# rdesc/autorally

Measured on AMD Instinct MI355X. Metric: trajectory rollouts/s per MPPI solve, higher is better.
Workload: dtype f32

## Files before the change

autorally_amd/capi.py:

```python
import ctypes as C
import os

import numpy as np

HERE = os.path.dirname(os.path.abspath(__file__))
LIB_PATH = os.environ.get("MPPI_LIB_PATH") or os.path.join(HERE, "libmppi_hip.so")
MAX_LAYERS = 8

OK, ERR_INVALID, ERR_NO_DEVICE, ERR_HIP, ERR_STATE, ERR_UNSUPPORTED = range(6)


class Config(C.Structure):
    _fields_ = [
        ("device", C.c_int),
        ("num_rollouts", C.c_int),
        ("num_timesteps", C.c_int),
        ("hz", C.c_int),
        ("optimization_stride", C.c_int),
        ("gamma", C.c_float),
        ("num_iters", C.c_int),
        ("n_layers", C.c_int),
        ("layers", C.c_int * MAX_LAYERS),
        ("exploration_std", C.c_float * 2),
        ("init_control", C.c_float * 2),
# ... 5 lines not shown


class CostParams(C.Structure):
    _fields_ = [(n, C.c_float) for n in (
        "desired_speed", "speed_coeff", "track_coeff", "max_slip_ang", "slip_penalty", "track_slop",
        "crash_coeff", "steering_coeff", "throttle_coeff", "boundary_threshold", "discount")] + [
        ("l1_cost", C.c_int)]


class StageTimes(C.Structure):
    _fields_ = [("n_solves", C.c_int), ("noise_ms", C.c_float), ("rollout_ms", C.c_float),
                ("weights_ms", C.c_float), ("reduction_ms", C.c_float), ("total_ms", C.c_float)]


SYMBOLS = [
    "mppi_abi_version", "mppi_strerror", "mppi_last_error", "mppi_device_count", "mppi_create",
    "mppi_destroy", "mppi_set_nn_params", "mppi_update_model", "mppi_set_control_limits",
    "mppi_set_costmap", "mppi_set_costmap_transform", "mppi_set_costmap_channel", "mppi_set_cost_params", "mppi_reset_controls",
    "mppi_set_control_seq", "mppi_get_control_seq", "mppi_set_control_hist", "mppi_get_control_hist",
    "mppi_savitsky_golay", "mppi_slide_control_seq", "mppi_seed", "mppi_set_noise", "mppi_generate_noise",
    "mppi_compute_control", "mppi_control_ticks", "mppi_compute_control_async", "mppi_synchronize",
    "mppi_compute_control_batch_async", "mppi_compute_control_batch", "mppi_control_ticks_batch", "mppi_get_results",
    "mppi_get_applied_controls", "mppi_rollout_only", "mppi_nominal_traj", "mppi_nominal_traj_pair",
    "mppi_set_bf_params", "mppi_set_ddp_weights", "mppi_debug_cost_raster", "mppi_compute_feedback_gains", "mppi_get_feedback_gains",
    "mppi_enable_stage_timing", "mppi_reset_stage_times", "mppi_get_stage_times",
    "mppi_rollout_variant", "mppi_set_rollout_variant", "mppi_debug_dynamics",
    "mppi_debug_inject_handover_fault", "mppi_compute_feedback_gains_pair", "mppi_set_host_threads",
    "mppi_debug_capture_iterations", "mppi_debug_get_iterations", "mppi_set_wait_timeout", "mppi_debug_form_candidates",
    "mppi_debug_set_chained_ticks", "mppi_debug_min_cost",
    "mppi_arm", "mppi_arm_batch", "mppi_disarm", "mppi_is_armed", "mppi_debug_launch_info",
    "mppi_trace_rollouts", "mppi_top_rollouts",
    "mppi_compute_feedback_gains_batch", "mppi_debug_ddp_info", "mppi_debug_device_tanhf",
    "mppi_nominal_traj_batch", "mppi_debug_nominal_info",
]

ABI2_SYMBOLS = ("mppi_debug_inject_handover_fault", "mppi_savitsky_golay", "mppi_set_costmap_transform",
                "mppi_compute_control_batch", "mppi_compute_control_batch_async", "mppi_control_ticks_batch",
                "mppi_nominal_traj_pair")
ABI3_SYMBOLS = ("mppi_compute_feedback_gains_pair", "mppi_set_host_threads")
ABI4_SYMBOLS = ("mppi_debug_capture_iterations", "mppi_debug_get_iterations", "mppi_set_wait_timeout", "mppi_debug_form_candidates")
ABI5_SYMBOLS = ("mppi_debug_set_chained_ticks", "mppi_debug_min_cost", "mppi_arm", "mppi_arm_batch", "mppi_disarm",
                "mppi_is_armed")

UNVERSIONED_SYMBOLS = ("mppi_debug_launch_info", "mppi_trace_rollouts", "mppi_top_rollouts",
                       "mppi_compute_feedback_gains_batch", "mppi_debug_ddp_info", "mppi_debug_device_tanhf",
                       "mppi_nominal_traj_batch", "mppi_debug_nominal_info")

_lib = None


class MppiError(RuntimeError):
    def __init__(self, status, msg):
        super().__init__("mppi status %d: %s" % (status, msg))
        self.status = status


def lib():
    global _lib
    if _lib is None:
        if not os.path.exists(LIB_PATH):
            raise RuntimeError("libmppi_hip.so is missing: run `python -m autorally_amd.build` "
                               "or __graft_entry__.build() first")
        L = C.CDLL(LIB_PATH)
        fp = C.POINTER(C.c_float)
        hp = C.c_void_p
        L.mppi_abi_version.restype = C.c_int
        L.mppi_strerror.restype = C.c_char_p
        L.mppi_strerror.argtypes = [C.c_int]
        L.mppi_last_error.restype = C.c_char_p
        L.mppi_last_error.argtypes = [hp]
        L.mppi_device_count.restype = C.c_int
        L.mppi_create.argtypes = [C.POINTER(Config), C.POINTER(hp)]
        L.mppi_destroy.argtypes = [hp]
        L.mppi_set_nn_params.argtypes = [hp, fp, C.c_size_t]
        L.mppi_update_model.argtypes = [hp, C.POINTER(C.c_int), C.c_int, fp, C.c_size_t]
        L.mppi_set_control_limits.argtypes = [hp, fp, fp]
        L.mppi_set_costmap.argtypes = [hp, C.c_int, C.c_int, fp, fp, fp, fp]
        L.mppi_set_costmap_transform.argtypes = [hp, fp, fp, fp]
        L.mppi_set_costmap_channel.argtypes = [hp, C.c_int, fp, C.c_size_t]
# ... 38 lines not shown
        v3 = L.mppi_abi_version() >= 3
        if v3:
            L.mppi_compute_feedback_gains_pair.argtypes = [hp, fp, fp, fp, hp, fp, fp, fp]
            L.mppi_set_host_threads.argtypes = [C.c_int]
        v4 = L.mppi_abi_version() >= 4
        if v4:
            L.mppi_debug_capture_iterations.argtypes = [hp, C.c_int]
            L.mppi_debug_get_iterations.argtypes = [hp, fp, fp, fp]
            L.mppi_set_wait_timeout.argtypes = [hp, C.c_double]
            L.mppi_debug_form_candidates.argtypes = [hp, C.POINTER(C.c_char_p), C.c_int]
        v5 = L.mppi_abi_version() >= 5
        if v5:
            L.mppi_debug_set_chained_ticks.argtypes = [hp, C.c_int]
            L.mppi_debug_min_cost.argtypes = [hp, C.c_int, C.POINTER(C.c_int)]
            L.mppi_arm.argtypes = [hp, C.c_double]
            L.mppi_arm_batch.argtypes = [C.POINTER(hp), C.c_int, C.c_double]
            L.mppi_disarm.argtypes = [hp]
            L.mppi_is_armed.argtypes = [hp]
        if hasattr(L, "mppi_debug_launch_info"):
            L.mppi_debug_launch_info.argtypes = [hp, C.POINTER(C.c_int), C.POINTER(C.c_int)]
        if hasattr(L, "mppi_trace_rollouts"):
            ip = C.POINTER(C.c_int)
            L.mppi_trace_rollouts.argtypes = [hp, ip, C.c_int, fp, fp, fp, fp, ip]
            L.mppi_top_rollouts.argtypes = [hp, C.c_int, ip]
        if hasattr(L, "mppi_compute_feedback_gains_batch"):
            fpp = C.POINTER(fp)
            L.mppi_compute_feedback_gains_batch.argtypes = [C.POINTER(hp), fp, fpp, fpp, C.c_int]
            L.mppi_debug_ddp_info.argtypes = [hp, C.POINTER(C.c_int)]
            L.mppi_debug_device_tanhf.argtypes = [C.c_int, fp, fp, C.c_size_t]
        if hasattr(L, "mppi_nominal_traj_batch"):
            fpp = C.POINTER(fp)
            L.mppi_nominal_traj_batch.argtypes = [C.POINTER(hp), fp, fpp, fpp, C.c_int]
            L.mppi_debug_nominal_info.argtypes = [hp, C.POINTER(C.c_int)]
        for s in SYMBOLS:
            if (v2 or s not in ABI2_SYMBOLS) and (v3 or s not in ABI3_SYMBOLS) and (v4 or s not in ABI4_SYMBOLS) and \
                    (v5 or s not in ABI5_SYMBOLS) and s not in UNVERSIONED_SYMBOLS:
                getattr(L, s)
        _lib = L
    return _lib


def _fp(a):
    return a.ctypes.data_as(C.POINTER(C.c_float))


def _f32(a, shape=None):
    a = np.ascontiguousarray(a, dtype=np.float32)
    if shape is not None:
        a = a.reshape(shape)
    return a


def make_config_struct(cfg, device=0):
    c = Config()
    c.device = int(device)
    c.num_rollouts = int(cfg["K"])
    c.num_timesteps = int(cfg["T"])
    c.hz = int(cfg["hz"])
    c.optimization_stride = int(cfg["opt_stride"])
    c.gamma = float(cfg["gamma"])
    c.num_iters = int(cfg.get("num_iters", 1))
    layers = [] if cfg.get("bf_W") is not None else [int(x) for x in cfg["layers"]]
    c.n_layers = len(layers)
    for i, v in enumerate(layers):
        c.layers[i] = v
    for i in range(2):
# ... 140 lines not shown
        self._ck(self.L.mppi_debug_min_cost(self.h, int(on), C.byref(got)))
        return bool(got.value)

    def arm(self, max_wait_s=0.01):
        self._ck(self.L.mppi_arm(self.h, float(max_wait_s)))

    def disarm(self):
        self._ck(self.L.mppi_disarm(self.h))

    def is_armed(self):
        return bool(self.L.mppi_is_armed(self.h))

    def debug_launch_info(self):
        n, g = C.c_int(-1), C.c_int(-1)
        self._ck(self.L.mppi_debug_launch_info(self.h, C.byref(n), C.byref(g)))
        return n.value, g.value

    def compute_control_async(self, state):
        self._ck(self.L.mppi_compute_control_async(self.h, _fp(_f32(state, (7,)))))

    def synchronize(self):
        self._ck(self.L.mppi_synchronize(self.h))

    def get_results(self, with_vectors=True):
        U = np.zeros((self.T, 2), dtype=np.float32)
        tc = C.c_float()
        costs = np.zeros(self.K, dtype=np.float32) if with_vectors else None
        w = np.zeros(self.K, dtype=np.float32) if with_vectors else None
        self._ck(self.L.mppi_get_results(self.h, _fp(U), C.byref(tc),
                                         _fp(costs) if with_vectors else None,
                                         _fp(w) if with_vectors else None))
        return dict(U=U, traj_cost=tc.value, costs=costs, w=w)

    def get_applied_controls(self):
        V = np.zeros((self.K, self.T, 2), dtype=np.float32)
        self._ck(self.L.mppi_get_applied_controls(self.h, _fp(V), V.size))
        return V

    def trace_rollouts(self, ks, with_costs=True):
        ks = np.ascontiguousarray(ks, dtype=np.int32).reshape(-1)
        n = ks.size
        out = dict(states=np.zeros((n, self.T, 7), np.float32), controls=np.zeros((n, self.T, 2), np.float32),
                   first_crash=np.zeros(n, np.int32))
        if with_costs:
            out.update(step_costs=np.zeros((n, self.T), np.float32), costs=np.zeros(n, np.float32))
        ip = C.POINTER(C.c_int)
        self._ck(self.L.mppi_trace_rollouts(self.h, ks.ctypes.data_as(ip), n, _fp(out["states"]), _fp(out["controls"]),
                                            _fp(out["step_costs"]) if with_costs else None,
                                            _fp(out["costs"]) if with_costs else None, out["first_crash"].ctypes.data_as(ip)))
        return out

    def top_rollouts(self, n):
        ks = np.zeros(int(n), np.int32)
        self._ck(self.L.mppi_top_rollouts(self.h, int(n), ks.ctypes.data_as(C.POINTER(C.c_int))))
        return ks

    def rollout_only(self, state):
        costs = np.zeros(self.K, dtype=np.float32)
        self._ck(self.L.mppi_rollout_only(self.h, _fp(_f32(state, (7,))), _fp(costs)))
        return costs

    def nominal_traj(self, state):
        ss = np.zeros((self.T, 7), dtype=np.float32)
        cs = np.zeros((self.T, 2), dtype=np.float32)
        self._ck(self.L.mppi_nominal_traj(self.h, _fp(_f32(state, (7,))), _fp(ss), _fp(cs)))
        return ss, cs
# ... 186 lines not shown
```

autorally_amd/csrc/abi_host.hip:

```cpp
#include "abi_internal.hpp"

#include <stdexcept>

using namespace mppi;
using namespace mppi_abi;

namespace mppi_abi {

class HostHelper {
 public:
  ~HostHelper()
  {
    if (!th_.joinable()) return;
    {
      std::lock_guard<std::mutex> lk(mu_);
      quit_ = true;
      wake_ = true;
    }
    cv_.notify_one();
    th_.join();
  }
  void arm()
  {
    std::call_once(started_, [this] { th_ = std::thread([this] { loop(); }); });
// ... 530 lines not shown
  for (int at = 0; at < n; at += kMaxFleet) {
    const int m = std::min(kMaxFleet, n - at);
    const int rcm = ddp_fleet_launch(handles + at, states + (size_t)MPPI_STATE_DIM * at, xs.data() + at, us.data() + at, m);
    if (rcm == MPPI_ERR_HIP) return rcm;
    if (rcm && !rc) rc = rcm;
  }
  return rc;
}

int mppi_debug_ddp_info(const mppi_handle *h, int *on_device)
{
  if (!h || !on_device) return MPPI_ERR_INVALID;
  *on_device = h->ddp_on_device;
  return MPPI_OK;
}

int mppi_debug_device_tanhf(int device, const float *in, float *out, size_t n)
{
  if (device < 0 || !in || !out || n == 0) return MPPI_ERR_INVALID;
  hipDeviceProp_t prop;
  if (hipGetDeviceProperties(&prop, device) != hipSuccess || strncmp(prop.gcnArchName, "gfx950", 6) != 0) return MPPI_ERR_NO_DEVICE;
  if (ensure_device(device) != hipSuccess) return MPPI_ERR_HIP;
  float *d_in = nullptr, *d_out = nullptr;
  hipError_t e = hipMalloc(reinterpret_cast<void **>(&d_in), sizeof(float) * n);
  if (e == hipSuccess) e = hipMalloc(reinterpret_cast<void **>(&d_out), sizeof(float) * n);
  if (e == hipSuccess) e = hipMemcpy(d_in, in, sizeof(float) * n, hipMemcpyHostToDevice);
  if (e == hipSuccess) e = launch_device_tanhf(d_in, d_out, n, nullptr);
  if (e == hipSuccess) e = hipMemcpy(out, d_out, sizeof(float) * n, hipMemcpyDeviceToHost);
  if (d_in) (void)hipFree(d_in);
  if (d_out) (void)hipFree(d_out);
  return e == hipSuccess ? MPPI_OK : MPPI_ERR_HIP;
}

int mppi_set_host_threads(int n)
{
  if (n < 1 || n > 2) return MPPI_ERR_INVALID;
  g_host_threads.store(n, std::memory_order_relaxed);
  if (n >= 2) host_helper().arm();
  return MPPI_OK;
}

int mppi_get_feedback_gains(mppi_handle *h, float *feedback, float *feedforward, float *state_traj,
                            float *control_traj, float *total_cost)
{
  if (!h) return MPPI_ERR_INVALID;
  if (!h->have_ddp) return fail(h, MPPI_ERR_STATE, "mppi_compute_feedback_gains has not succeeded yet");
  const DdpResult &r = h->ddp;
  if (feedback) memcpy(feedback, r.feedback.data(), sizeof(float) * r.feedback.size());
  if (feedforward) memcpy(feedforward, r.feedforward.data(), sizeof(float) * r.feedforward.size());
  if (state_traj) memcpy(state_traj, r.x.data(), sizeof(float) * r.x.size());
  if (control_traj) memcpy(control_traj, r.u.data(), sizeof(float) * r.u.size());
  if (total_cost) *total_cost = r.total_cost;
  return MPPI_OK;
}

}
```

autorally_amd/csrc/abi_solve.hip:

```cpp
#include "abi_internal.hpp"

using namespace mppi;
using namespace mppi_abi;

namespace mppi_abi {

std::mutex g_batch_mu;
hipStream_t g_batch_stream[64] = {};
hipStream_t batch_stream(int device)
{
  if (device < 0 || device >= 64) return nullptr;
  std::lock_guard<std::mutex> lk(g_batch_mu);
  if (!g_batch_stream[device] &&
      hipStreamCreateWithFlags(&g_batch_stream[device], hipStreamNonBlocking) != hipSuccess)
    g_batch_stream[device] = nullptr;
  return g_batch_stream[device];
}

hipError_t arg_block_create(ArgBlock &b, size_t slot_bytes)
{
  b.slot = (slot_bytes + 255) & ~(size_t)255;
  hipError_t e = hipMalloc(reinterpret_cast<void **>(&b.d), b.slot);
  if (e == hipSuccess) e = hipHostMalloc(reinterpret_cast<void **>(&b.h), b.slot * ArgBlock::kRing, hipHostMallocDefault);
  for (int i = 0; i < ArgBlock::kRing && e == hipSuccess; i++) e = hipEventCreateWithFlags(&b.ev[i], hipEventDisableTiming);
// ... 1150 lines not shown
}

int mppi_rollout_only(mppi_handle *h, const float state[MPPI_STATE_DIM], float *costs)
{
  int rc = check_ready(h);
  if (rc) return rc;
  if (!state || !costs) return fail(h, MPPI_ERR_INVALID, "NULL argument");
  DISARM(h);
  HIPCHK(h, hipSetDevice(h->cfg.device));
  rc = recover_timed_out(h);
  if (rc) return rc;
  rc = mppi_synchronize(h);
  if (rc) return rc;
  OWN(h);
  rc = upload_controls_if_dirty(h, h->stream);
  if (rc) return rc;
  float *noise = nullptr;
  bool in_kernel = false;
  rc = eps_source(h, Eps::Single, 0, &noise, &in_kernel, nullptr);
  if (rc) return rc;
  h->explicit_iters = 0;
  forget_solve_state(h);
  RolloutArgs a;
  fill_rollout_args(h, state, noise, a);
  if (in_kernel) use_inline_noise(h, a);
  rc = launch_rollout(h, a);
  if (rc) return rc;
  note_solve_state(h, state, false);
  HIPCHK(h, hipMemcpyAsync(costs, h->d_costs, sizeof(float) * h->K, hipMemcpyDeviceToHost, h->stream));
  HIPCHK(h, hipStreamSynchronize(h->stream));
  return MPPI_OK;
}

int mppi_debug_capture_iterations(mppi_handle *h, int on)
{
  if (!h) return MPPI_ERR_INVALID;
  DISARM(h);
  int rc = mppi_synchronize(h);
  if (rc) return rc;
  if (on && !h->d_cap) {
    HIPCHK(h, hipSetDevice(h->cfg.device));
    HIPCHK(h, hipMalloc(&h->d_cap, sizeof(float) * (size_t)h->cfg.num_iters * (2 * (size_t)h->T + h->K)));
  }
  h->capture = on != 0;
  h->cap_valid = false;
  return MPPI_OK;
}

int mppi_debug_get_iterations(mppi_handle *h, float *U_raw, float *costs, float *V)
{
  if (!h) return MPPI_ERR_INVALID;
  int rc = mppi_synchronize(h);
  if (rc) return rc;
  if (!h->cap_valid) return fail(h, MPPI_ERR_STATE, "no captured solve (mppi_debug_capture_iterations, then a solve on this handle alone)");
  if (V && !h->cap_explicit) return fail(h, MPPI_ERR_STATE, "applied controls of every iteration exist for explicit-noise solves only");
  const int iters = h->cfg.num_iters, T = h->T, K = h->K;
  HIPCHK(h, hipSetDevice(h->cfg.device));
  OWN(h);
  HIPCHK(h, hipStreamSynchronize(h->stream));
  const size_t rec = 2 * (size_t)T + K;
  std::vector<float> buf((size_t)iters * rec);
  HIPCHK(h, hipMemcpy(buf.data(), h->d_cap, sizeof(float) * buf.size(), hipMemcpyDeviceToHost));
  for (int it = 0; it < iters; it++) {
    if (U_raw) {
      float *u = U_raw + (size_t)it * 2 * T;
      if (it < iters - 1) memcpy(u, buf.data() + (size_t)it * rec, sizeof(float) * 2 * (size_t)T);
// ... 77 lines not shown
```

autorally_amd/csrc/mppi_device.hpp:

```cpp
#pragma once

#include <hip/hip_runtime.h>
#include <stdint.h>

namespace mppi {

constexpr int kStateDim = 7;
constexpr int kControlDim = 2;
constexpr int kNetIn = 6;
constexpr int kNetOut = 4;
constexpr int kRolloutsPerWave = 16;

struct CostArgs {
  float desired_speed, speed_coeff, track_coeff, max_slip_ang, slip_penalty, track_slop;
  float crash_coeff, steering_coeff, throttle_coeff, boundary_threshold;
  float crash_cost_discounted;
  int l1_cost;
  float r_c1[3], r_c2[3], trs[3];
  int affine;
  int need_control_cost;
  int map_w, map_h;
  const float *map;
};

// ... 126 lines not shown
  return r;
}

__device__ __forceinline__ float tanh_fast(float x)
{
  const float e = __builtin_amdgcn_exp2f(x * 2.88539008177792681472f);
  const float r = __builtin_amdgcn_rcpf(e + 1.0f);
  return fmaf(-2.0f, r, 1.0f);
}

constexpr float kTanhScale = 2.88539008177792681472f;
__device__ __forceinline__ float tanh_bias(float z, float bs)
{
  const float e = __builtin_amdgcn_exp2f(fmaf(z, kTanhScale, bs));
  const float r = __builtin_amdgcn_rcpf(e + 1.0f);
  return fmaf(-2.0f, r, 1.0f);
}

typedef float f32x2 __attribute__((ext_vector_type(2)));
typedef float f32x4 __attribute__((ext_vector_type(4)));
__device__ __forceinline__ f32x2 tanh_bias2(f32x2 z, f32x2 bs)
{
  const f32x2 y = __builtin_elementwise_fma(z, f32x2{kTanhScale, kTanhScale}, bs);
  f32x2 e;
  e.x = __builtin_amdgcn_exp2f(y.x);
  e.y = __builtin_amdgcn_exp2f(y.y);
  const f32x2 d = e + f32x2{1.0f, 1.0f};
  f32x2 r;
  r.x = __builtin_amdgcn_rcpf(d.x);
  r.y = __builtin_amdgcn_rcpf(d.y);
  return __builtin_elementwise_fma(f32x2{-2.0f, -2.0f}, r, f32x2{1.0f, 1.0f});
}

__device__ __forceinline__ void sincos_fast(float x, float &sn, float &cs)
{
  const double xd = (double)x;
  const double q = rint(xd * 0.63661977236758134308);
  double rd = fma(-q, 1.5707963267948966, xd);
  rd = fma(-q, 6.123233995736766e-17, rd);
  const float r = (float)rd;
  const float r2 = r * r;
  const float ps = fmaf(fmaf(-1.9515295891e-4f, r2, 8.3321608736e-3f), r2, -1.6666654611e-1f);
  const float s0 = fmaf(r * r2, ps, r);
  const float pc = fmaf(fmaf(2.443315711809948e-5f, r2, -1.388731625493765e-3f), r2, 4.166664568298827e-2f);
  const float c0 = fmaf(r2 * r2, pc, fmaf(r2, -0.5f, 1.0f));
  const int qi = (int)q;
  const float a = (qi & 1) ? c0 : s0;
  const float b = (qi & 1) ? s0 : c0;
  sn = (qi & 2) ? -a : a;
  cs = ((qi + 1) & 2) ? -b : b;
}

template <bool AFFINE>
__device__ __forceinline__ unsigned texel_index(const CostArgs &c, float x, float y)
{
  float u = fmaf(c.r_c1[0], x, c.r_c2[0] * y) + c.trs[0];
  float v = fmaf(c.r_c1[1], x, c.r_c2[1] * y) + c.trs[1];
  if (!AFFINE) {
    const float w = fmaf(c.r_c1[2], x, c.r_c2[2] * y) + c.trs[2];
    u = u / w;
    v = v / w;
  }
  float fi = floorf(u * (float)c.map_w);
  float fj = floorf(v * (float)c.map_h);
  fi = fminf(fmaxf(fi, 0.0f), (float)(c.map_w - 1));
  fj = fminf(fmaxf(fj, 0.0f), (float)(c.map_h - 1));
// ... 136 lines not shown
```

autorally_amd/csrc/mppi_kernels.hpp:

```cpp
#pragma once
#include "mppi_device.hpp"

#include <hip/hip_ext.h>
#include <atomic>
#include <type_traits>

namespace mppi {

extern thread_local hipEvent_t tl_kernel_start, tl_kernel_stop;
#define MPPI_LAUNCH_ROLLOUT(kern, grid, block, lds, stream, ...)                                                   \
  do {                                                                                                             \
    if (::mppi::tl_kernel_start != nullptr)                                                                        \
      hipExtLaunchKernelGGL(kern, grid, block, lds, stream, ::mppi::tl_kernel_start, ::mppi::tl_kernel_stop, 0,    \
                            __VA_ARGS__);                                                                          \
    else                                                                                                           \
      hipLaunchKernelGGL(kern, grid, block, lds, stream, __VA_ARGS__);                                             \
  } while (0)

template <class F>
inline hipError_t dispatch_cost_flags(bool affine, bool ctrl, F &&f)
{
  if (affine && !ctrl) return f(std::true_type{}, std::false_type{});
  if (affine && ctrl) return f(std::true_type{}, std::true_type{});
  if (!affine && !ctrl) return f(std::false_type{}, std::false_type{});
// ... 197 lines not shown
  int *first_crash;
  int n, K, T;
  float nu[2], u_lo[2], u_hi[2], dt;
  int negate_yaw_der;
  CostArgs cost;
};
bool trace_image_in_lds(const NetDesc &net);
hipError_t launch_rollout_trace(const NetDesc &net, const TraceArgs &a, hipStream_t stream);
hipError_t launch_rollout_trace_bf(const TraceArgs &a, hipStream_t stream);

struct TailLaunch {
  const float *costs, *V, *hist;
  float *U, *w, *scal, *res, *slid;
  unsigned *counter;
  int K, T, last_iter, slide_stride;
  unsigned seq;
  float gamma, init0, init1;
  unsigned long long *ug = nullptr;
  int no_device_copy = 0;
  float *hist_out = nullptr;
  unsigned long long *gx = nullptr, *gpart = nullptr;
  unsigned epoch = 0, poll_ticks = 0;
  int fault = 0;
  const unsigned long long *min_cost = nullptr;
  unsigned min_cost_tag = 0;
};
bool tail_is_stream(int K);
constexpr int kTailExchangeGranules = 3 * 64 + 32 * 16 + 32 * 64;
hipError_t launch_solve_tail(const TailLaunch &l, hipStream_t stream);
hipError_t launch_solve_tail_batch(const TailLaunch *l, int n, hipStream_t stream);
size_t solve_tail_fleet_arg_bytes();
void fill_solve_tail_fleet(void *dst, const TailLaunch *l, int n);
hipError_t launch_solve_tail_fleet(const TailLaunch *l, int n, const void *d_args, hipStream_t stream);
hipError_t launch_debug_cost(const CostArgs &c, float x, float y, float heading, int width_m, int height_m,
                             int ppm, float *out, hipStream_t stream);
hipError_t launch_slide(float *in, int T, int stride, float init0, float init1, hipStream_t stream);
hipError_t launch_kt_to_tk(const float *src, float *dst, int K, int T, hipStream_t stream);
hipError_t launch_tk_to_kt(const float *src, float *dst, int K, int T, hipStream_t stream);

hipError_t launch_noise(const uint32_t *rng_in, uint32_t *rng_out, const uint32_t *jump, int K, int T,
                        int L, int C, float *eps, hipStream_t stream);
struct NoiseFleetDesc {
  const uint32_t *rng_in;
  uint32_t *rng_out;
  const uint32_t *jump;
  float *eps;
  int K, T, L, C;
};
hipError_t launch_noise_fleet(const NoiseFleetDesc *h_desc, const NoiseFleetDesc *d_desc, int n, hipStream_t stream);
hipError_t launch_noise_init(uint32_t *rng, int K, const uint32_t base[6], const uint32_t *sub,
                             int sub_bits, const uint32_t *one, uint64_t offset, hipStream_t stream);

struct DdpFleetArgs {
  const float *theta;
  const float *wimg;
  const float *in;
  float *out, *work;
  int T, negate_yaw_der;
  int img_lds;
  float dt;
  float u_lo[2], u_hi[2], Q[7], R[2], Qf[7];
  NetDesc net;
};
__host__ __device__ inline int ddp_fleet_hidden(const NetDesc &net)
{
  int s = 0;
// ... 27 lines not shown
```

autorally_amd/csrc/solve_kernels.hip:

```cpp
#include "mppi_device.hpp"
#include "mppi_kernels.hpp"


namespace mppi {


#ifdef MPPI_TAIL_STAMPS
__device__ unsigned long long g_tail_stamps[16];
#define TSTAMP(i)                                                                                   \
  do {                                                                                              \
    if (block == T / 2 && threadIdx.x == 0) {                                                       \
      unsigned long long t__;                                                                       \
      asm volatile("s_memrealtime %0\n\ts_waitcnt lgkmcnt(0)" : "=s"(t__)::"memory");               \
      g_tail_stamps[i] = t__;                                                                       \
    }                                                                                               \
  } while (0)
#else
#define TSTAMP(i) do { } while (0)
#endif
#ifndef MPPI_TAIL_THREADS
#define MPPI_TAIL_THREADS 512
#endif
constexpr int kTailThreads = MPPI_TAIL_THREADS;
constexpr int kRedChunk = 4096;

__device__ __forceinline__ float wave_min(float v) { return wave_reduce<true>(v); }
__device__ __forceinline__ float wave_sum(float v) { return wave_reduce<false>(v); }
template <bool MIN>
__device__ __forceinline__ float block_reduce(float v, float *red4)
{
  const int lane = threadIdx.x & 63, wv = threadIdx.x >> 6;
  v = wave_reduce<MIN>(v);
  if (lane == 0) red4[wv] = v;
  __syncthreads();
  float r = red4[0];
#pragma unroll
  for (int i = 1; i < kTailThreads / 64; i++) r = MIN ? fminf(r, red4[i]) : r + red4[i];
  return r;
}

__device__ __forceinline__ void publish_entry(float *res, int entry, float v0, float v1, unsigned seq)
{
  const f32x4 v = {v0, __uint_as_float(seq), v1, __uint_as_float(seq)};
  float *p = res + 4 * (size_t)entry;
  asm volatile("global_store_dwordx4 %0, %1, off sc0 sc1" ::"v"(p), "v"(v) : "memory");
}

__device__ __forceinline__ unsigned long long make_granule(unsigned epoch, float v)
{
  return ((unsigned long long)epoch << 32) | (unsigned long long)__float_as_uint(v);
}
__device__ __forceinline__ void store_granule(unsigned long long *g, unsigned epoch, float v)
{
  __hip_atomic_store(g, make_granule(epoch, v), __ATOMIC_RELAXED, __HIP_MEMORY_SCOPE_AGENT);
}

struct TailArgs {
  const float *costs;
  const float *V;
  float *U;
  const float *hist;
  float *w;
  float *scal;
  float *res;
  int no_device_copy;
  float *hist_out;
  unsigned long long *ug;
  unsigned *counter;
  int K, T;
  float gamma;
  float *slid;
// ... 79 lines not shown
      a.slid[2 * T + tid] = hv;
    }
  }
}

__device__ __forceinline__ void solve_tail_body(const TailArgs &a, const int block, const float *V, const float *costs_p, const int K,
                                                const int T)
{
  constexpr int kGS = 68, kPlane = (kRedChunk / 64) * kGS;
  __shared__ __attribute__((aligned(16))) float tile[2][kPlane];
  __shared__ __attribute__((aligned(16))) float wtile[kPlane];
  __shared__ float redm[kTailThreads / 64], reds[kTailThreads / 64], redt[kTailThreads / 64];
  __shared__ int is_last;
  extern __shared__ __attribute__((aligned(16))) float dyn[];
  float *partial = dyn;
  const int tid = threadIdx.x;
  const bool extra = (block == T);
  const int t = extra ? 0 : block;
  constexpr int base = 0;
  const int n = K;
  TSTAMP(0);

  const float *row = V + ((size_t)t * K + base) * 2;
  constexpr int kPre = kRedChunk / 2 / kTailThreads;
  float4 pre[kPre];
  {
    const float4 *src0 = reinterpret_cast<const float4 *>(row);
#pragma unroll
    for (int i = 0; i < kPre; i++) {
      const int q = tid + i * kTailThreads;
      pre[i] = (q < n / 2) ? src0[q] : make_float4(0, 0, 0, 0);
    }
  }
  float eta;
  {
    constexpr int kCostV = kRedChunk / 4 / kTailThreads;
    const float4 *c4 = reinterpret_cast<const float4 *>(costs_p);
    const int K4 = K / 4;
    float4 cv[kCostV];
#pragma unroll
    for (int i = 0; i < kCostV; i++) {
      const int q = i * kTailThreads + tid;
      cv[i] = (q < K4) ? c4[q] : make_float4(INFINITY, INFINITY, INFINITY, INFINITY);
    }
    float m = INFINITY;
    TSTAMP(1);
#pragma unroll
    for (int i = 0; i < kCostV; i++) m = fminf(fminf(m, fminf(cv[i].x, cv[i].y)), fminf(cv[i].z, cv[i].w));
    TSTAMP(2);
    const float beta = block_reduce<true>(m, redm);
    TSTAMP(3);
    float part = 0.0f;
#pragma unroll
    for (int i = 0; i < kCostV; i++) {
      const int q = i * kTailThreads + tid;
      if (q < K4) {
        const float e0 = expf(-a.gamma * (cv[i].x - beta));
        const float e1 = expf(-a.gamma * (cv[i].y - beta));
        const float e2 = expf(-a.gamma * (cv[i].z - beta));
        const float e3 = expf(-a.gamma * (cv[i].w - beta));
        cv[i] = make_float4(e0, e1, e2, e3);
        part += (e0 + e1) + (e2 + e3);
      }
    }
    TSTAMP(4);
    eta = block_reduce<false>(part, reds);
    TSTAMP(5);
    if (extra) {
      float tc = 0.0f;
#pragma unroll
      for (int i = 0; i < kCostV; i++) {
        const int q = i * kTailThreads + tid;
        if (q < K4) {
          reinterpret_cast<float4 *>(a.w)[q] = cv[i];
          tc += cv[i].x * cv[i].x / eta;
          tc += cv[i].y * cv[i].y / eta;
          tc += cv[i].z * cv[i].z / eta;
          tc += cv[i].w * cv[i].w / eta;
        }
      }
      const float traj = block_reduce<false>(tc, redt);
      if (tid == 0) {
        __hip_atomic_store(&a.scal[0], beta, __ATOMIC_RELAXED, __HIP_MEMORY_SCOPE_AGENT);
        __hip_atomic_store(&a.scal[1], eta, __ATOMIC_RELAXED, __HIP_MEMORY_SCOPE_AGENT);
        __hip_atomic_store(&a.scal[2], traj, __ATOMIC_RELAXED, __HIP_MEMORY_SCOPE_AGENT);
        if (a.last_iter) {
          publish_entry(a.res, T, beta, eta, a.seq);
          publish_entry(a.res, T + 1, traj, 0.0f, a.seq);
        }
      }
    } else {
#pragma unroll
      for (int i = 0; i < kCostV; i++) {
        const int q = i * kTailThreads + tid;
        const int kl = 4 * q - base;
        if (q < K4 && kl >= 0 && kl < n)
          *reinterpret_cast<float4 *>(&wtile[(kl >> 6) * kGS + (kl & 63)]) =
              make_float4(cv[i].x / eta, cv[i].y / eta, cv[i].z / eta, cv[i].w / eta);
      }
    }
  }

  const int G = K / 64;
  if (!extra) {
#pragma unroll
    for (int i = 0; i < kPre; i++) {
      const int q = tid + i * kTailThreads;
      if (q < n / 2) {
        const int kk = 2 * q;
        const int o = (kk >> 6) * kGS + (kk & 63);
        *reinterpret_cast<float2 *>(&tile[0][o]) = make_float2(pre[i].x, pre[i].z);
        *reinterpret_cast<float2 *>(&tile[1][o]) = make_float2(pre[i].y, pre[i].w);
      }
    }
    TSTAMP(6);
    __syncthreads();
    TSTAMP(7);
    for (int c = tid; c < (n / 64) * 2; c += kTailThreads) {
      const int ml = c >> 1, j = c & 1;
      const float4 *p4 = reinterpret_cast<const float4 *>(&tile[j][ml * kGS]);
      const float4 *w4 = reinterpret_cast<const float4 *>(&wtile[ml * kGS]);
      float acc = 0.0f;
#pragma unroll
      for (int i = 0; i < 16; i++) {
        const float4 wv = w4[i], pv = p4[i];
        acc = fmaf(wv.x, pv.x, acc);
        acc = fmaf(wv.y, pv.y, acc);
        acc = fmaf(wv.z, pv.z, acc);
        acc = fmaf(wv.w, pv.w, acc);
      }
      partial[j * G + ml] = acc;
    }
    TSTAMP(8);
    __syncthreads();
  }
  float u = 0.0f;
  if (tid < 2 && !extra) {
    const float *pj = partial + tid * G;
    int mm = 0;
    if ((G & 3) == 0) {
      for (; mm + 32 <= G; mm += 32) {
        float4 v[8];
#pragma unroll
        for (int i = 0; i < 8; i++) v[i] = *reinterpret_cast<const float4 *>(pj + mm + 4 * i);
#pragma unroll
        for (int i = 0; i < 8; i++) { u += v[i].x; u += v[i].y; u += v[i].z; u += v[i].w; }
      }
    }
    for (; mm < G; mm++) u += pj[mm];
    if (a.last_iter) store_granule(a.ug + t * 2 + tid, a.seq, u);
    else a.U[t * 2 + tid] = u;
  }
  if (tid < 64) {
    const float u1 = __shfl(u, 1);
    TSTAMP(9);
    if (tid == 0 && !extra && a.last_iter) publish_entry(a.res, t, u, u1, a.seq);
    TSTAMP(10);
  }
  tail_arrive_and_smooth(a, K, T, (unsigned)(T + 1), is_last, dyn);
}

#ifdef MPPI_TAIL_STAMPS
// ... 337 lines not shown
  }
  SSTAMP(9);
  __syncthreads();
  float u = 0.0f;
  if (tid < 2) {
    const float *pj = partial + tid * G;
    int mm = 0;
    if ((G & 3) == 0 && G >= 32) {
      float4 v[8], w[8];
#pragma unroll
      for (int i = 0; i < 8; i++) v[i] = *reinterpret_cast<const float4 *>(pj + 4 * i);
      for (; mm + 32 <= G; mm += 32) {
        const int nx = (mm + 64 <= G) ? mm + 32 : mm;
#pragma unroll
        for (int i = 0; i < 8; i++) w[i] = *reinterpret_cast<const float4 *>(pj + nx + 4 * i);
#pragma unroll
        for (int i = 0; i < 8; i++) { u += v[i].x; u += v[i].y; u += v[i].z; u += v[i].w; }
#pragma unroll
        for (int i = 0; i < 8; i++) v[i] = w[i];
      }
    }
    for (; mm < G; mm++) u += pj[mm];
    if (a.last_iter) store_granule(a.ug + t * 2 + tid, a.seq, u);
    else a.U[t * 2 + tid] = u;
  }
  if (tid < 64) {
    const float u1 = __shfl(u, 1);
    if (tid == 0 && a.last_iter) publish_entry(a.res, t, u, u1, a.seq);
    SSTAMP(10);
  }
  tail_arrive_and_smooth(a, K, T, (unsigned)T, is_last, img);
}

__global__ __launch_bounds__(kTailThreads) void solve_tail_kernel(const float *V, const float *costs, const int K, const int T,
                                                                  const TailArgs a)
{
  solve_tail_body(a, (int)blockIdx.x, V, costs, K, T);
}

template <int NB>
struct TailBatchArgs {
  TailArgs inst[NB];
};
template <int NB>
__global__ __launch_bounds__(kTailThreads) void solve_tail_batch_kernel(const TailBatchArgs<NB> b)
{
#define MPPI_TAIL_BODY(A)                                                   \
  do {                                                                      \
    if ((int)blockIdx.x > (A).T) return;                                    \
    solve_tail_body((A), (int)blockIdx.x, (A).V, (A).costs, (A).K, (A).T);    \
  } while (0)
  MPPI_BATCH_DISPATCH(NB, b, MPPI_TAIL_BODY);
#undef MPPI_TAIL_BODY
}

__global__ __launch_bounds__(kTailThreads) void solve_tail_fleet_kernel(const TailArgs *__restrict__ inst, const int n)
{
  if ((int)blockIdx.y >= n) return;
  TailArgs a = inst[blockIdx.y];
  if ((int)blockIdx.x > a.T) return;
  a.costs = load_global_ptr(inst[blockIdx.y].costs); a.V = load_global_ptr(inst[blockIdx.y].V); a.U = load_global_ptr(inst[blockIdx.y].U); a.hist = load_global_ptr(inst[blockIdx.y].hist); a.w = load_global_ptr(inst[blockIdx.y].w);
  a.scal = load_global_ptr(inst[blockIdx.y].scal); a.res = load_global_ptr(inst[blockIdx.y].res); a.hist_out = load_global_ptr(inst[blockIdx.y].hist_out); a.ug = load_global_ptr(inst[blockIdx.y].ug);
  a.counter = load_global_ptr(inst[blockIdx.y].counter); a.slid = load_global_ptr(inst[blockIdx.y].slid); a.min_cost = load_global_ptr(inst[blockIdx.y].min_cost);
  solve_tail_body(a, (int)blockIdx.x, a.V, a.costs, a.K, a.T);
}

__global__ void slide_kernel(float *__restrict__ in, int T, int stride, float init0, float init1)
{
  extern __shared__ float buf[];
  float *U = in, *hist = in + 2 * T;
  for (int i = threadIdx.x; i < 2 * T; i += blockDim.x) buf[i] = U[i];
  float hold = 0.0f;
  if (threadIdx.x < 4) hold = hist[threadIdx.x];
  const float hold2 = __shfl(hold, (threadIdx.x + 2) & 63);
  __syncthreads();
  if (threadIdx.x < 4) {
    const int i = threadIdx.x;
    float hv;
    if (stride == 1) hv = (i < 2) ? hold2 : buf[i - 2];
    else hv = buf[(stride - 2) + i];
    hist[i] = hv;
  }
  for (int i = threadIdx.x; i < 2 * T; i += blockDim.x) {
    const int r = i >> 1, j = i & 1;
    float v;
    if (r < T - stride) v = buf[(r + stride) * 2 + j];
    else v = j ? init1 : init0;
    U[i] = v;
  }
// ... 35 lines not shown
                                                        int height_m, int ppm, float *__restrict__ out)
{
  const int x_idx = blockIdx.x * 16 + (threadIdx.x & 15);
  const int y_idx = blockIdx.y * 16 + (threadIdx.x >> 4);
  const int W = width_m * ppm, H = height_m * ppm;
  float x_pos = (float)x_idx / (float)ppm;
  float y_pos = (float)y_idx / (float)ppm;
  x_pos -= (float)width_m * 0.5f;
  y_pos -= (float)height_m * 0.5f;
  x_pos += x;
  y_pos += y;
  float cost = c.map[c.affine ? texel_index<true>(c, x_pos, y_pos) : texel_index<false>(c, x_pos, y_pos)];
  if (x_idx < W && (H - y_idx) < H) {
    float sh, ch;
    sincos_fast(heading, sh, ch);
    const float dx = x_pos - x, dy = y_pos - y;
    const float xt = fmaf(ch, dx, sh * dy);
    const float yt = fmaf(-sh, dx, ch * dy);
    const float dist = (float)(0.25 * (double)fabsf(xt) + (double)fabsf(yt));
    if ((double)dist < .15 && xt > 0.0f) cost = ((double)dist < .1 && (double)xt > 0.05) ? 1.0f : 0.0f;
    const int idx = (H - (y_idx + 1)) * W + x_idx;
    if (idx > 0 && idx < W * H) out[idx] = cost;
  }
}

hipError_t launch_debug_cost(const CostArgs &c, float x, float y, float heading, int width_m, int height_m,
                             int ppm, float *out, hipStream_t stream)
{
  const dim3 grid((width_m * ppm - 1) / 16 + 1, (height_m * ppm - 1) / 16 + 1);
  hipLaunchKernelGGL(debug_cost_kernel, grid, dim3(256), 0, stream, c, x, y, heading, width_m, height_m, ppm, out);
  return hipGetLastError();
}

static size_t tail_dyn_bytes(int K, int T)
{
  return ((size_t)(K / 64) * 2 + (size_t)(T + 4) * 2 + (size_t)T * 2) * sizeof(float);
}

static TailArgs fill_tail(const TailLaunch &l)
{
  TailArgs a;
  a.slid = l.slid; a.slide_stride = l.slide_stride; a.init0 = l.init0; a.init1 = l.init1;
  a.costs = l.costs; a.V = l.V; a.U = l.U; a.hist = l.hist; a.w = l.w; a.scal = l.scal; a.res = l.res; a.ug = l.ug;
  a.no_device_copy = l.no_device_copy; a.hist_out = l.hist_out; a.min_cost = l.min_cost; a.min_cost_tag = l.min_cost_tag;
  a.counter = l.counter;
  a.K = l.K; a.T = l.T; a.gamma = l.gamma; a.last_iter = l.last_iter; a.seq = l.seq;
  return a;
}

bool tail_is_stream(int K) { return K > kRedChunk; }

hipError_t launch_solve_tail(const TailLaunch &l, hipStream_t stream)
{
  const TailArgs a = fill_tail(l);
  const int K = l.K, T = l.T;
  const int C = (K + kRedChunk - 1) / kRedChunk;
  if (tail_is_stream(K)) {
    if (C > kMaxChunks || !l.gx || !l.gpart || l.epoch == 0 || l.poll_ticks == 0) return hipErrorInvalidValue;
    StreamTailArgs sa;
    sa.a = a;
    sa.gx = l.gx; sa.gpart = l.gpart; sa.epoch = l.epoch; sa.poll_ticks = l.poll_ticks; sa.fault = l.fault;
    if ((size_t)(K / 64) * 2 + (size_t)(T + 4) * 2 + (size_t)T * 2 > (size_t)3 * kRedChunk) return hipErrorInvalidValue;
    const int grid = ((C + 7) & ~7) + 8 * ((T + 7) / 8) * C;
    hipLaunchKernelGGL(solve_tail_stream_kernel, dim3(grid), dim3(kTailThreads), 0, stream, a.V, a.costs, K, T, sa);
    return hipGetLastError();
  }
// ... 82 lines not shown
```

include/mppi_hip.h:

```cpp
#ifndef MPPI_HIP_H_
#define MPPI_HIP_H_

#include <stddef.h>
#include <stdint.h>

#ifdef __cplusplus
extern "C" {
#endif

#define MPPI_ABI_VERSION 5
#define MPPI_STATE_DIM 7
#define MPPI_CONTROL_DIM 2
#define MPPI_MAX_LAYERS 8

enum {
  MPPI_OK = 0,
  MPPI_ERR_INVALID = 1,
  MPPI_ERR_NO_DEVICE = 2,
  MPPI_ERR_HIP = 3,
  MPPI_ERR_STATE = 4,
  MPPI_ERR_UNSUPPORTED = 5
};

typedef struct mppi_handle mppi_handle;
// ... 110 lines not shown
                                     const float *target_state_seq_b, const float *target_control_seq_b);

int mppi_compute_feedback_gains_batch(mppi_handle *const *handles, const float *states, const float *const *target_state_seqs,
                                      const float *const *target_control_seqs, int n);
int mppi_debug_ddp_info(const mppi_handle *h, int *on_device);
int mppi_debug_device_tanhf(int device, const float *in, float *out, size_t n);

int mppi_set_host_threads(int n);

int mppi_debug_cost_raster(mppi_handle *h, float x, float y, float heading, int width_m, int height_m,
                           int ppm, float *out, size_t n);

int mppi_enable_stage_timing(mppi_handle *h, int on);
int mppi_reset_stage_times(mppi_handle *h);
int mppi_get_stage_times(mppi_handle *h, mppi_stage_times *out);
const char *mppi_rollout_variant(const mppi_handle *h);
int mppi_set_rollout_variant(mppi_handle *h, const char *name);

int mppi_debug_dynamics(mppi_handle *h, int n, const float *states, const float *controls, float *ders);

int mppi_debug_inject_handover_fault(mppi_handle *h, int wave, int spin_budget);

int mppi_debug_capture_iterations(mppi_handle *h, int on);
int mppi_debug_get_iterations(mppi_handle *h, float *U_raw, float *costs, float *V);

int mppi_debug_form_candidates(const mppi_handle *h, const char **names, int max_n);

int mppi_debug_set_chained_ticks(mppi_handle *h, int on);

int mppi_debug_min_cost(mppi_handle *h, int on, int *from_rollout);

int mppi_debug_launch_info(mppi_handle *h, int *instances, int *gated);

int mppi_set_wait_timeout(mppi_handle *h, double seconds);

#ifdef __cplusplus
}
#endif
#endif
```

Before: 105.8 million.

## Overlap tile staging with beta reduction and speed up solve-tail arithmetic

The solve tail kernel now writes the prefetched control-noise tile into shared memory between posting and reading the block-min reduction, so the staging overlaps the barrier wait. The scalar expf weighting is replaced by a paired f32x2 exp for non-positive arguments built on the hardware exp2 with a split log2e constant. The weighted-sum inner loop preloads shared-memory operands ahead of the FMAs under sched_barrier fences, and the tail kernels get a min-waves-per-SIMD launch bound. Debug entry points are added to check the tail and the custom exp against expf, since the exp path may differ slightly in accuracy and the launch bound adds register pressure.

Result: no change. 106.4 million (median of 2 runs) (+0.6%).

```diff
diff --git a/autorally_amd/capi.py b/autorally_amd/capi.py
--- a/autorally_amd/capi.py
+++ b/autorally_amd/capi.py
@@ -61,6 +61,7 @@
     "mppi_trace_rollouts", "mppi_top_rollouts",
     "mppi_compute_feedback_gains_batch", "mppi_debug_ddp_info", "mppi_debug_device_tanhf",
     "mppi_nominal_traj_batch", "mppi_debug_nominal_info",
+    "mppi_debug_solve_tail", "mppi_debug_tail_arith",
 ]
 
 ABI2_SYMBOLS = ("mppi_debug_inject_handover_fault", "mppi_savitsky_golay", "mppi_set_costmap_transform",
@@ -73,7 +74,8 @@
 
 UNVERSIONED_SYMBOLS = ("mppi_debug_launch_info", "mppi_trace_rollouts", "mppi_top_rollouts",
                        "mppi_compute_feedback_gains_batch", "mppi_debug_ddp_info", "mppi_debug_device_tanhf",
-                       "mppi_nominal_traj_batch", "mppi_debug_nominal_info")
+                       "mppi_nominal_traj_batch", "mppi_debug_nominal_info",
+                       "mppi_debug_solve_tail", "mppi_debug_tail_arith")
 
 _lib = None
 
@@ -178,6 +180,10 @@
             fpp = C.POINTER(fp)
             L.mppi_nominal_traj_batch.argtypes = [C.POINTER(hp), fp, fpp, fpp, C.c_int]
             L.mppi_debug_nominal_info.argtypes = [hp, C.POINTER(C.c_int)]
+        if hasattr(L, "mppi_debug_solve_tail"):
+            L.mppi_debug_solve_tail.argtypes = [hp, fp, fp, fp, fp]
+        if hasattr(L, "mppi_debug_tail_arith"):
+            L.mppi_debug_tail_arith.argtypes = [C.c_int, fp, fp, fp, C.c_size_t]
         for s in SYMBOLS:
             if (v2 or s not in ABI2_SYMBOLS) and (v3 or s not in ABI3_SYMBOLS) and (v4 or s not in ABI4_SYMBOLS) and \
                     (v5 or s not in ABI5_SYMBOLS) and s not in UNVERSIONED_SYMBOLS:
@@ -384,6 +390,13 @@
                                          _fp(w) if with_vectors else None))
         return dict(U=U, traj_cost=tc.value, costs=costs, w=w)
 
+    def debug_solve_tail(self, costs, V):
+        costs = _f32(costs, (self.K,))
+        V = _f32(V, (self.T, self.K, 2))
+        beta, eta = C.c_float(), C.c_float()
+        self._ck(self.L.mppi_debug_solve_tail(self.h, _fp(costs), _fp(V), C.byref(beta), C.byref(eta)))
+        return beta.value, eta.value
+
     def get_applied_controls(self):
         V = np.zeros((self.K, self.T, 2), dtype=np.float32)
         self._ck(self.L.mppi_get_applied_controls(self.h, _fp(V), V.size))
diff --git a/autorally_amd/csrc/abi_host.hip b/autorally_amd/csrc/abi_host.hip
--- a/autorally_amd/csrc/abi_host.hip
+++ b/autorally_amd/csrc/abi_host.hip
@@ -586,6 +586,22 @@
   return e == hipSuccess ? MPPI_OK : MPPI_ERR_HIP;
 }
 
+int mppi_debug_tail_arith(int device, const float *x, float *fast, float *plain, size_t n)
+{
+  if (device < 0 || !x || !fast || !plain || n == 0 || n % 4 != 0) return MPPI_ERR_INVALID;
+  hipDeviceProp_t prop;
+  if (hipGetDeviceProperties(&prop, device) != hipSuccess || strncmp(prop.gcnArchName, "gfx950", 6) != 0) return MPPI_ERR_NO_DEVICE;
+  if (ensure_device(device) != hipSuccess) return MPPI_ERR_HIP;
+  float *d = nullptr;
+  hipError_t e = hipMalloc(reinterpret_cast<void **>(&d), sizeof(float) * 3 * n);
+  if (e == hipSuccess) e = hipMemcpy(d, x, sizeof(float) * n, hipMemcpyHostToDevice);
+  if (e == hipSuccess) e = launch_tail_arith(d, d + n, d + 2 * n, n, nullptr);
+  if (e == hipSuccess) e = hipMemcpy(fast, d + n, sizeof(float) * n, hipMemcpyDeviceToHost);
+  if (e == hipSuccess) e = hipMemcpy(plain, d + 2 * n, sizeof(float) * n, hipMemcpyDeviceToHost);
+  if (d) (void)hipFree(d);
+  return e == hipSuccess ? MPPI_OK : MPPI_ERR_HIP;
+}
+
 int mppi_set_host_threads(int n)
 {
   if (n < 1 || n > 2) return MPPI_ERR_INVALID;
diff --git a/autorally_amd/csrc/abi_solve.hip b/autorally_amd/csrc/abi_solve.hip
--- a/autorally_amd/csrc/abi_solve.hip
+++ b/autorally_amd/csrc/abi_solve.hip
@@ -1206,6 +1206,37 @@
   return MPPI_OK;
 }
 
+int mppi_debug_solve_tail(mppi_handle *h, const float *costs, const float *V, float *beta, float *eta)
+{
+  if (!h) return MPPI_ERR_INVALID;
+  if (!costs || !V) return fail(h, MPPI_ERR_INVALID, "NULL argument");
+  if (tail_is_stream(h->K)) return fail(h, MPPI_ERR_UNSUPPORTED, "mppi_debug_solve_tail: the one-chunk tail serves K <= 4096");
+  DISARM(h);
+  HIPCHK(h, hipSetDevice(h->cfg.device));
+  int rc = recover_timed_out(h);
+  if (rc) return rc;
+  rc = mppi_synchronize(h);
+  if (rc) return rc;
+  OWN(h);
+  rc = begin_solves(&h, 1, h->stream, false);
+  if (rc) return rc;
+  h->explicit_iters = 0;
+  float *vbuf = h->d_gen[h->gen_cur];
+  h->v_buf = vbuf;
+  HIPCHK(h, hipMemcpyAsync(h->d_costs, costs, sizeof(float) * (size_t)h->K, hipMemcpyHostToDevice, h->stream));
+  HIPCHK(h, hipMemcpyAsync(vbuf, V, sizeof(float) * 2 * (size_t)h->K * h->T, hipMemcpyHostToDevice, h->stream));
+  next_tail_epoch(h);
+  const TailLaunch l = tail_launch(h, vbuf, true);
+  HIPCHK(h, launch_solve_tail(l, h->stream));
+  h->slid_valid = wants_slid_copy(h);
+  h->pending = true;
+  h->pending_timed = false;
+  rc = wait_pending(h);
+  if (beta) *beta = h->baseline;
+  if (eta) *eta = h->eta;
+  return rc;
+}
+
 int mppi_debug_capture_iterations(mppi_handle *h, int on)
 {
   if (!h) return MPPI_ERR_INVALID;
diff --git a/autorally_amd/csrc/mppi_device.hpp b/autorally_amd/csrc/mppi_device.hpp
--- a/autorally_amd/csrc/mppi_device.hpp
+++ b/autorally_amd/csrc/mppi_device.hpp
@@ -182,6 +182,27 @@
   return __builtin_elementwise_fma(f32x2{-2.0f, -2.0f}, r, f32x2{1.0f, 1.0f});
 }
 
+__device__ __forceinline__ f32x2 exp_nonpos2(f32x2 x)
+{
+  constexpr float kLog2eHi = __builtin_bit_cast(float, 0x3fb8aa3bu), kLog2eLo = __builtin_bit_cast(float, 0x32a5705fu);
+  constexpr float kUnderflow = __builtin_bit_cast(float, 0xc2ce8ed0u);
+  const f32x2 hi = {kLog2eHi, kLog2eHi}, lo = {kLog2eLo, kLog2eLo};
+  f32x2 t = x * hi;
+  f32x2 r = __builtin_elementwise_fma(x, hi, -t);
+  f32x2 n;
+  n.x = __builtin_rintf(t.x);
+  n.y = __builtin_rintf(t.y);
+  r = __builtin_elementwise_fma(x, lo, r);
+  t = t - n;
+  t = t + r;
+  f32x2 e;
+  e.x = __builtin_ldexpf(__builtin_amdgcn_exp2f(t.x), (int)n.x);
+  e.y = __builtin_ldexpf(__builtin_amdgcn_exp2f(t.y), (int)n.y);
+  e.x = (kUnderflow > x.x) ? 0.0f : e.x;
+  e.y = (kUnderflow > x.y) ? 0.0f : e.y;
+  return e;
+}
+
 __device__ __forceinline__ void sincos_fast(float x, float &sn, float &cs)
 {
   const double xd = (double)x;
diff --git a/autorally_amd/csrc/mppi_kernels.hpp b/autorally_amd/csrc/mppi_kernels.hpp
--- a/autorally_amd/csrc/mppi_kernels.hpp
+++ b/autorally_amd/csrc/mppi_kernels.hpp
@@ -253,6 +253,7 @@
 size_t solve_tail_fleet_arg_bytes();
 void fill_solve_tail_fleet(void *dst, const TailLaunch *l, int n);
 hipError_t launch_solve_tail_fleet(const TailLaunch *l, int n, const void *d_args, hipStream_t stream);
+hipError_t launch_tail_arith(const float *x, float *fast, float *plain, size_t n, hipStream_t stream);
 hipError_t launch_debug_cost(const CostArgs &c, float x, float y, float heading, int width_m, int height_m,
                              int ppm, float *out, hipStream_t stream);
 hipError_t launch_slide(float *in, int T, int stride, float init0, float init1, hipStream_t stream);
diff --git a/autorally_amd/csrc/solve_kernels.hip b/autorally_amd/csrc/solve_kernels.hip
--- a/autorally_amd/csrc/solve_kernels.hip
+++ b/autorally_amd/csrc/solve_kernels.hip
@@ -22,21 +22,32 @@
 #define MPPI_TAIL_THREADS 512
 #endif
 constexpr int kTailThreads = MPPI_TAIL_THREADS;
+constexpr int kTailWavesPerSimd = 2 * (kTailThreads / 64) / 4;
 constexpr int kRedChunk = 4096;
 
 __device__ __forceinline__ float wave_min(float v) { return wave_reduce<true>(v); }
 __device__ __forceinline__ float wave_sum(float v) { return wave_reduce<false>(v); }
 template <bool MIN>
-__device__ __forceinline__ float block_reduce(float v, float *red4)
+__device__ __forceinline__ void block_reduce_put(float v, float *red4)
 {
   const int lane = threadIdx.x & 63, wv = threadIdx.x >> 6;
   v = wave_reduce<MIN>(v);
   if (lane == 0) red4[wv] = v;
+}
+template <bool MIN>
+__device__ __forceinline__ float block_reduce_get(const float *red4)
+{
   __syncthreads();
   float r = red4[0];
 #pragma unroll
   for (int i = 1; i < kTailThreads / 64; i++) r = MIN ? fminf(r, red4[i]) : r + red4[i];
   return r;
+}
+template <bool MIN>
+__device__ __forceinline__ float block_reduce(float v, float *red4)
+{
+  block_reduce_put<MIN>(v, red4);
+  return block_reduce_get<MIN>(red4);
 }
 
 __device__ __forceinline__ void publish_entry(float *res, int entry, float v0, float v1, unsigned seq)
@@ -182,6 +193,18 @@
       pre[i] = (q < n / 2) ? src0[q] : make_float4(0, 0, 0, 0);
     }
   }
+  auto stage_row = [&]() {
+#pragma unroll
+    for (int i = 0; i < kPre; i++) {
+      const int q = tid + i * kTailThreads;
+      if (q < n / 2) {
+        const int kk = 2 * q;
+        const int o = (kk >> 6) * kGS + (kk & 63);
+        *reinterpret_cast<float2 *>(&tile[0][o]) = make_float2(pre[i].x, pre[i].z);
+        *reinterpret_cast<float2 *>(&tile[1][o]) = make_float2(pre[i].y, pre[i].w);
+      }
+    }
+  };
   float eta;
   {
     constexpr int kCostV = kRedChunk / 4 / kTailThreads;
@@ -198,19 +221,21 @@
 #pragma unroll
     for (int i = 0; i < kCostV; i++) m = fminf(fminf(m, fminf(cv[i].x, cv[i].y)), fminf(cv[i].z, cv[i].w));
     TSTAMP(2);
-    const float beta = block_reduce<true>(m, redm);
+    block_reduce_put<true>(m, redm);
+    if (!extra) stage_row();
+    TSTAMP(6);
+    const float beta = block_reduce_get<true>(redm);
     TSTAMP(3);
     float part = 0.0f;
+    const f32x2 beta2 = {beta, beta}, ngamma2 = {-a.gamma, -a.gamma};
 #pragma unroll
     for (int i = 0; i < kCostV; i++) {
       const int q = i * kTailThreads + tid;
       if (q < K4) {
-        const float e0 = expf(-a.gamma * (cv[i].x - beta));
-        const float e1 = expf(-a.gamma * (cv[i].y - beta));
-        const float e2 = expf(-a.gamma * (cv[i].z - beta));
-        const float e3 = expf(-a.gamma * (cv[i].w - beta));
-        cv[i] = make_float4(e0, e1, e2, e3);
-        part += (e0 + e1) + (e2 + e3);
+        const f32x2 e01 = exp_nonpos2(ngamma2 * (f32x2{cv[i].x, cv[i].y} - beta2));
+        const f32x2 e23 = exp_nonpos2(ngamma2 * (f32x2{cv[i].z, cv[i].w} - beta2));
+        cv[i] = make_float4(e01.x, e01.y, e23.x, e23.y);
+        part += (e01.x + e01.y) + (e23.x + e23.y);
       }
     }
     TSTAMP(4);
@@ -253,17 +278,6 @@
 
   const int G = K / 64;
   if (!extra) {
-#pragma unroll
-    for (int i = 0; i < kPre; i++) {
-      const int q = tid + i * kTailThreads;
-      if (q < n / 2) {
-        const int kk = 2 * q;
-        const int o = (kk >> 6) * kGS + (kk & 63);
-        *reinterpret_cast<float2 *>(&tile[0][o]) = make_float2(pre[i].x, pre[i].z);
-        *reinterpret_cast<float2 *>(&tile[1][o]) = make_float2(pre[i].y, pre[i].w);
-      }
-    }
-    TSTAMP(6);
     __syncthreads();
     TSTAMP(7);
     for (int c = tid; c < (n / 64) * 2; c += kTailThreads) {
@@ -271,13 +285,22 @@
       const float4 *p4 = reinterpret_cast<const float4 *>(&tile[j][ml * kGS]);
       const float4 *w4 = reinterpret_cast<const float4 *>(&wtile[ml * kGS]);
       float acc = 0.0f;
+      constexpr int kAhead = 12;
+      float4 wv[16], pv[16];
+#pragma unroll
+      for (int i = 0; i < kAhead; i++) { wv[i] = w4[i]; pv[i] = p4[i]; }
+      __builtin_amdgcn_sched_barrier(0);
 #pragma unroll
       for (int i = 0; i < 16; i++) {
-        const float4 wv = w4[i], pv = p4[i];
-        acc = fmaf(wv.x, pv.x, acc);
-        acc = fmaf(wv.y, pv.y, acc);
-        acc = fmaf(wv.z, pv.z, acc);
-        acc = fmaf(wv.w, pv.w, acc);
+        if (i == 16 - kAhead) {
+#pragma unroll
+          for (int r = kAhead; r < 16; r++) { wv[r] = w4[r]; pv[r] = p4[r]; }
+          __builtin_amdgcn_sched_barrier(0);
+        }
+        acc = fmaf(wv[i].x, pv[i].x, acc);
+        acc = fmaf(wv[i].y, pv[i].y, acc);
+        acc = fmaf(wv[i].z, pv[i].z, acc);
+        acc = fmaf(wv[i].w, pv[i].w, acc);
       }
       partial[j * G + ml] = acc;
     }
@@ -681,7 +704,7 @@
   tail_arrive_and_smooth(a, K, T, (unsigned)T, is_last, img);
 }
 
-__global__ __launch_bounds__(kTailThreads) void solve_tail_kernel(const float *V, const float *costs, const int K, const int T,
+__global__ __launch_bounds__(kTailThreads, kTailWavesPerSimd) void solve_tail_kernel(const float *V, const float *costs, const int K, const int T,
                                                                   const TailArgs a)
 {
   solve_tail_body(a, (int)blockIdx.x, V, costs, K, T);
@@ -692,7 +715,7 @@
   TailArgs inst[NB];
 };
 template <int NB>
-__global__ __launch_bounds__(kTailThreads) void solve_tail_batch_kernel(const TailBatchArgs<NB> b)
+__global__ __launch_bounds__(kTailThreads, kTailWavesPerSimd) void solve_tail_batch_kernel(const TailBatchArgs<NB> b)
 {
 #define MPPI_TAIL_BODY(A)                                                   \
   do {                                                                      \
@@ -703,7 +726,7 @@
 #undef MPPI_TAIL_BODY
 }
 
-__global__ __launch_bounds__(kTailThreads) void solve_tail_fleet_kernel(const TailArgs *__restrict__ inst, const int n)
+__global__ __launch_bounds__(kTailThreads, kTailWavesPerSimd) void solve_tail_fleet_kernel(const TailArgs *__restrict__ inst, const int n)
 {
   if ((int)blockIdx.y >= n) return;
   TailArgs a = inst[blockIdx.y];
@@ -805,6 +828,26 @@
   return hipGetLastError();
 }
 
+__global__ __launch_bounds__(256) void tail_arith_kernel(const float4 *__restrict__ x, float4 *__restrict__ fast, float4 *__restrict__ plain,
+                                                         size_t n4)
+{
+  const size_t i = (size_t)blockIdx.x * 256 + threadIdx.x;
+  if (i >= n4) return;
+  const float4 v = x[i];
+  const f32x2 a = exp_nonpos2(f32x2{v.x, v.y}), b = exp_nonpos2(f32x2{v.z, v.w});
+  fast[i] = make_float4(a.x, a.y, b.x, b.y);
+  plain[i] = make_float4(expf(v.x), expf(v.y), expf(v.z), expf(v.w));
+}
+
+hipError_t launch_tail_arith(const float *x, float *fast, float *plain, size_t n, hipStream_t stream)
+{
+  if (n == 0 || n % 4 != 0) return hipErrorInvalidValue;
+  const size_t n4 = n / 4;
+  hipLaunchKernelGGL(tail_arith_kernel, dim3((unsigned)((n4 + 255) / 256)), dim3(256), 0, stream, reinterpret_cast<const float4 *>(x),
+                     reinterpret_cast<float4 *>(fast), reinterpret_cast<float4 *>(plain), n4);
+  return hipGetLastError();
+}
+
 static size_t tail_dyn_bytes(int K, int T)
 {
   return ((size_t)(K / 64) * 2 + (size_t)(T + 4) * 2 + (size_t)T * 2) * sizeof(float);
diff --git a/include/mppi_hip.h b/include/mppi_hip.h
--- a/include/mppi_hip.h
+++ b/include/mppi_hip.h
@@ -166,6 +166,10 @@
 
 int mppi_debug_launch_info(mppi_handle *h, int *instances, int *gated);
 
+int mppi_debug_solve_tail(mppi_handle *h, const float *costs, const float *V, float *beta, float *eta);
+
+int mppi_debug_tail_arith(int device, const float *x, float *fast, float *plain, size_t n);
+
 int mppi_set_wait_timeout(mppi_handle *h, double seconds);
 
 #ifdef __cplusplus
```
